# jinhan/tacotron2-vae

Measured on AMD Instinct MI355X. Metric: mel-frames/s (train step, batch=6, 80-mel), higher is better.
Workload: dtype f32; 1 GPU; configs[1]: Tacotron2-VAE fp32 train step (fwd+loss+bwd+clip+Adam), B=6/GPU fixed shape T_in=84 T_out=400, dropout on, random-init seed 1234; step_mode=hip-graph replay, decoder_forward=persistent, decoder_backward=persistent, startup_steps=43, global_batch=6, parallelism=dp1

## Files before the change

### tacotron2-vae_amd/csrc/conv_gemm.hip

```cpp
#include <stdlib.h>
#include <type_traits>
#include "t2v_common.h"
#include "t2v_kernels.h"
#include "t2v_coop.h"
#include "t2v_x3.h"


#define CG_BM 64
#define CG_BN 64
#define CG_BK 32

struct ConvGemmArgs {
    const float* W;
    const float* X;
    const float* dY;
    const float* bias;
    float* Y;
    float* stat_part;
    int B, Cin, T, M, KS;
};

template <int MODE, int KS>
__global__ __launch_bounds__(256) void k_conv_gemm(ConvGemmArgs a) {
    __shared__ float As[2][CG_BK][CG_BM + 1];
// ... 157 lines not shown
        if (second_ == 0u) return;
        if (tid == 0) __hip_atomic_store(a.ks_ctr + tile, 0u, __ATOMIC_RELAXED, __HIP_MEMORY_SCOPE_AGENT);
        const float* other = a.ks_part + (((1 - blockIdx.z) * ntile + tile) * 256 + tid) * (4 * NTW);
        float o[NTW][4];
#pragma unroll
        for (int n = 0; n < NTW; ++n)
#pragma unroll
            for (int r = 0; r < 4; ++r) o[n][r] = ld_sc1(other + 4 * n + r);
#pragma unroll
        for (int n = 0; n < NTW; ++n)
#pragma unroll
            for (int r = 0; r < 4; ++r) acc[n][r] += o[n][r];
    }
    float psum[4] = {0.f, 0.f, 0.f, 0.f}, psq[4] = {0.f, 0.f, 0.f, 0.f};
#pragma unroll
    for (int r = 0; r < 4; ++r) {
        const int m = m0 + 16 * wave + 4 * kq + r;
        if (m < a.M) {
            const float bv = a.bias ? a.bias[m] : 0.f;
            float* yrow = a.Y + ((size_t)bb * a.M + m) * a.T;
#pragma unroll
            for (int n = 0; n < NTW; ++n) {
                const int t = t0 + 16 * n + j;
                if (t < a.T) {
                    const float v = acc[n][r] + bv;
                    yrow[t] = v;
                    psum[r] += v;
                    psq[r] = fmaf(v, v, psq[r]);
                }
            }
        }
    }
    if (a.stat_part) {
#pragma unroll
        for (int r = 0; r < 4; ++r) {
            const float s1 = row16_sum(psum[r]), s2 = row16_sum(psq[r]);
            const int m = m0 + 16 * wave + 4 * kq + r;
            if (j == 0 && m < a.M) {
                float* dst = a.stat_part + ((size_t)blockIdx.x * a.M + m) * 2;
                dst[0] = s1;
                dst[1] = s2;
            }
        }
    }
}

template <int NTW>
__global__ __launch_bounds__(256) void k_conv5_fwd(ConvTiledArgs a) {
    constexpr int BN = 16 * NTW;
    constexpr int XW = BN + 4;
    constexpr int XS = BN == 32 ? 48 : BN <= 64 ? 80 : 112;
    constexpr int NX = (16 * XW + 255) / 256;
    __shared__ float As[2][CT_KT][CT_AS];
    __shared__ float Xs[2][16][XS];
    const int tid = threadIdx.x, wave = tid >> 6, lane = tid & 63;
    const int kq = lane >> 4, j = lane & 15;
    const int bb = blockIdx.x / a.tiles_per_item, t0 = (blockIdx.x % a.tiles_per_item) * BN;
    const int m0 = blockIdx.y * CT_BM;
    const int CK = a.Cin * 5;
    const int nkt_all = a.Cin / 16;
    const int kt0 = gridDim.z > 1 ? (int)blockIdx.z * (nkt_all / 2) : 0;
    const int nkt = gridDim.z > 1 ? (blockIdx.z == 0 ? nkt_all / 2 : nkt_all - nkt_all / 2) : nkt_all;

    const bool stamp = a.prof && tid == 0 && blockIdx.x == 0 && blockIdx.y == 0 && blockIdx.z == 0;
    if (stamp) { a.prof[0] = __builtin_readcyclecounter(); a.prof[2] = wall_clock64(); }
    float4 ra[5];
    float rx[NX];
    const int a_m = tid & 63, w4 = tid >> 6;
    const float* a_row = a.W + (size_t)min(m0 + a_m, a.M - 1) * CK + 4 * w4;
    int a_lds[20];
#pragma unroll
    for (int q = 0; q < 20; ++q) {
        const int k = 4 * w4 + 16 * (q >> 2) + (q & 3);
        const int c = k / 5, kx = k - 5 * c;
        a_lds[q] = (16 * kx + c) * CT_AS + a_m;
    }
    const float* x_item = a.X + (size_t)bb * a.Cin * a.T;
    int x_goff[NX], x_lds[NX];
    bool x_ok[NX];
#pragma unroll
    for (int i = 0; i < NX; ++i) {
        const int e = tid + 256 * i;
        const int c = min(e / XW, 15), jj = e - (e / XW) * XW;
        const int t = t0 - 2 + jj;
        x_ok[i] = e < 16 * XW && t >= 0 && t < a.T;
        x_goff[i] = c * a.T + min(max(t, 0), a.T - 1);
        x_lds[i] = e < 16 * XW ? c * XS + jj : -1;
    }
    auto load_one = [&](int kt, int q) {
        if (q < 5) {
            ra[q] = *(const float4*)(a_row + 80 * (kt0 + kt) + 16 * q);
        } else {
            const float v = x_item[(size_t)16 * (kt0 + kt) * a.T + x_goff[q - 5]];
            rx[q - 5] = x_ok[q - 5] ? v : 0.f;
        }
    };
    auto store_one = [&](int buf, int q) {
        if (q < 20) {
            const float4 v4 = ra[q >> 2];
            const float v = (q & 3) == 0 ? v4.x : (q & 3) == 1 ? v4.y : (q & 3) == 2 ? v4.z : v4.w;
            (&As[buf][0][0])[a_lds[q]] = v;
        } else if (q < 20 + NX) {
            if (x_lds[q - 20] >= 0) (&Xs[buf][0][0])[x_lds[q - 20]] = rx[q - 20];
        }
    };
    constexpr int NLOAD = 5 + NX, NSTORE = 20 + NX;
    constexpr int S_ST0 = 11;
    static_assert(NLOAD <= S_ST0 + 1 && NSTORE <= 3 * (20 - S_ST0), "side work must fit the k-steps");

    f32x4 acc[NTW];
#pragma unroll
    for (int n = 0; n < NTW; ++n) acc[n] = f32x4{0.f, 0.f, 0.f, 0.f};
#pragma unroll
    for (int q = 0; q < NLOAD; ++q) load_one(0, q);
#pragma unroll
    for (int q = 0; q < NSTORE; ++q) store_one(0, q);
    __syncthreads();
    for (int kt = 0; kt < nkt; ++kt) {
        const int buf = kt & 1;
        const int kn = min(kt + 1, nkt - 1);
        const float* ap = &As[buf][kq][16 * wave + j];
        const float* xp = &Xs[buf][kq][j];
        float av[2], bv[2][NTW];
        av[0] = ap[0];
#pragma unroll
        for (int n = 0; n < NTW; ++n) bv[0][n] = xp[16 * n];
#pragma unroll
        for (int s = 0; s < 20; ++s) {
            if (s < NLOAD) load_one(kn, s);
            if (s + 1 < 20) {
                av[(s + 1) & 1] = ap[4 * (s + 1) * CT_AS];
#pragma unroll
                for (int n = 0; n < NTW; ++n)
                    bv[(s + 1) & 1][n] = xp[4 * ((s + 1) & 3) * XS + 16 * n + ((s + 1) >> 2)];
            }
            __builtin_amdgcn_sched_barrier(0);
#pragma unroll
            for (int n = 0; n < NTW; ++n) acc[n] = mfma16x4(av[s & 1], bv[s & 1][n], acc[n]);
            __builtin_amdgcn_sched_barrier(0);
            if (s >= S_ST0) {
#pragma unroll
                for (int q = 3 * (s - S_ST0); q < 3 * (s - S_ST0) + 3; ++q) store_one(buf ^ 1, q);
                __builtin_amdgcn_sched_barrier(0);
            }
        }
        __syncthreads();
    }
    if (stamp) { a.prof[1] = __builtin_readcyclecounter(); a.prof[3] = wall_clock64(); }
    conv5_fwd_finish<NTW>(a, acc, bb, t0, m0);
}

#define CD_RING 3
#define CD_AS 84
__device__ float g_conv5_zero[4];

template <int NTW>
__global__ __launch_bounds__(256) void k_conv5_fwd_dma(ConvTiledArgs a) {
    constexpr int BN = 16 * NTW;
    constexpr int XW = BN + 4;
    constexpr int XS = BN == 32 ? 48 : BN <= 64 ? 80 : 112;
    constexpr int NXD = 16 * XS / 256;
    constexpr int G = 6 + NXD;
    constexpr int AST = CT_BM * CD_AS, STG = AST + 16 * XS;
    static_assert(16 * XS % 256 == 0 && AST % 256 == 0, "whole 64-lane requests");
    __shared__ __attribute__((aligned(16))) float lds_[CD_RING * STG];
    const unsigned lds0 = (unsigned)(unsigned long)(__attribute__((address_space(3))) void*)&lds_[0];
    const int tid = threadIdx.x, wave = __builtin_amdgcn_readfirstlane(tid >> 6), lane = tid & 63;
    const int kq = lane >> 4, j = lane & 15;
    const int bb = blockIdx.x / a.tiles_per_item, t0 = (blockIdx.x % a.tiles_per_item) * BN;
    const int m0 = blockIdx.y * CT_BM;
    const int CK = a.Cin * 5;
    const int nkt_all = a.Cin / 16;
    const int kt0 = gridDim.z > 1 ? (int)blockIdx.z * (nkt_all / 2) : 0;
    const int nkt = gridDim.z > 1 ? (blockIdx.z == 0 ? nkt_all / 2 : nkt_all - nkt_all / 2) : nkt_all;

    const bool stamp = a.prof && tid == 0 && blockIdx.x == 0 && blockIdx.y == 0 && blockIdx.z == 0;
    if (stamp) { a.prof[0] = __builtin_readcyclecounter(); a.prof[2] = wall_clock64(); }
    const float* a_ptr[6];
#pragma unroll
    for (int i = 0; i < 6; ++i) {
        const int u = 64 * min(wave + 4 * i, 20) + lane;
        const int row = u / 21, pc = u - 21 * row;
        a_ptr[i] = a.W + (size_t)min(m0 + row, a.M - 1) * CK + 80 * kt0 + 4 * min(pc, 19);
    }
    const float* x_ptr[NXD];
    size_t x_step[NXD];
#pragma unroll
    for (int i = 0; i < NXD; ++i) {
        const int e = 64 * (wave + 4 * i) + lane;
        const int c = e / XS, jj = e - c * XS;
        const int t = t0 - 2 + jj;
        const bool ok = jj < XW && t >= 0 && t < a.T;
        x_ptr[i] = ok ? a.X + ((size_t)bb * a.Cin + 16 * kt0 + c) * a.T + t : g_conv5_zero;
        x_step[i] = ok ? (size_t)16 * a.T : 0;
    }
    auto request = [&](unsigned dst, int q) {
        if (q < 5) {
            t2v_dma16(a_ptr[q], dst + 1024u * (unsigned)wave + 4096u * q);
            a_ptr[q] += 80;
        } else if (q == 5) {
            t2v_dma16(a_ptr[5], dst + 20480u);
            a_ptr[5] += 80;
        } else if (q < G) {
            t2v_dma4(x_ptr[q - 6], dst + 4u * AST + 256u * (unsigned)wave + 1024u * (q - 6));
            x_ptr[q - 6] += x_step[q - 6];
        }
    };

    f32x4 acc[NTW];
#pragma unroll
    for (int n = 0; n < NTW; ++n) acc[n] = f32x4{0.f, 0.f, 0.f, 0.f};
#pragma unroll
    for (int q = 0; q < G; ++q) request(lds0, q);
    if (nkt > 1) {
#pragma unroll
        for (int q = 0; q < G; ++q) request(lds0 + 4u * STG, q);
    }
    if (nkt > 1) t2v_wait_vmcnt<G>(); else t2v_wait_vmcnt<0>();
    __syncthreads();
    constexpr int CD_SYNC = 10;
    constexpr int TWO = G > 20 - CD_SYNC ? G - (20 - CD_SYNC) : 0;
    static_assert(G <= 2 * (20 - CD_SYNC) && (TWO == 0 || NTW >= 3), "a tile's requests fit the steps behind the barrier");
    const int lane_a = CD_AS * (16 * wave + j) + 5 * kq, lane_x = AST + kq * XS + j;
    float av[2], bv[2][NTW];
    auto fetch = [&](const float* ap, const float* xp, int s) {
        av[s & 1] = ap[20 * (s & 3) + (s >> 2)];
#pragma unroll
        for (int n = 0; n < NTW; ++n) bv[s & 1][n] = xp[4 * (s & 3) * XS + 16 * n + (s >> 2)];
    };
    auto tile = [&](auto more_c, const float* ap, const float* xp, const float* ap1, const float* xp1, unsigned dst2) {
        constexpr bool MORE = decltype(more_c)::value;
#pragma unroll
        for (int s = 0; s < 20; ++s) {
            if (s == CD_SYNC) {
                t2v_wait_vmcnt<0>();
                __syncthreads();
                __builtin_amdgcn_sched_barrier(0);
            }
            const int sr = s - CD_SYNC;
            const int q0 = !MORE || sr < 0 ? -1 : sr < TWO ? 2 * sr : sr + TWO;
            const int q1 = MORE && sr >= 0 && sr < TWO ? 2 * sr + 1 : -1;
#pragma unroll
            for (int n = 0; n < NTW; ++n) {
                acc[n] = mfma16x4(av[s & 1], bv[s & 1][n], acc[n]);
                __builtin_amdgcn_sched_barrier(0);
                if (n == 0) { if (s + 1 < 20) fetch(ap, xp, s + 1); else fetch(ap1, xp1, 0); }
                if (n == 1 && q0 >= 0 && q0 < G) request(dst2, q0);
                if (n == 2 && q1 >= 0) request(dst2, q1);
                __builtin_amdgcn_sched_barrier(0);
            }
        }
    };
    fetch(&lds_[lane_a], &lds_[lane_x], 0);
    int stg = 0;
    for (int kt = 0; kt < nkt; ++kt) {
        const int stg1 = stg == CD_RING - 1 ? 0 : stg + 1, stg2 = stg == 0 ? CD_RING - 1 : stg - 1;
        const float* ap = &lds_[stg * STG + lane_a];
        const float* xp = &lds_[stg * STG + lane_x];
        const float* ap1 = &lds_[stg1 * STG + lane_a];
        const float* xp1 = &lds_[stg1 * STG + lane_x];
        if (kt + 2 < nkt) tile(std::true_type{}, ap, xp, ap1, xp1, lds0 + 4u * (unsigned)(stg2 * STG));
        else tile(std::false_type{}, ap, xp, ap1, xp1, 0u);
        stg = stg1;
    }
    if (stamp) { a.prof[1] = __builtin_readcyclecounter(); a.prof[3] = wall_clock64(); }
    conv5_fwd_finish<NTW>(a, acc, bb, t0, m0);
}

template <int BT>
__global__ __launch_bounds__(256) void k_conv5_dw(ConvTiledArgs a) {
    constexpr int XW = BT + 4;
    constexpr int XS = (BT == 80) ? 100 : 116;
    constexpr int NA = BT / 16;
    constexpr int NX = (16 * XW + 255) / 256;
    __shared__ float As[2][BT][CT_AS];
    __shared__ float Xs[2][16][XS];
    const int tid = threadIdx.x, wave = tid >> 6, lane = tid & 63;
    const int kq = lane >> 4, j = lane & 15;
    const int c0 = blockIdx.x * 16, m0 = blockIdx.y * CT_BM;
    const int CK = a.Cin * 5;
    const int tiles = (a.T + BT - 1) / BT, nkt_all = a.B * tiles;
    const int per = (nkt_all + gridDim.z - 1) / gridDim.z;
    const int kt_lo = blockIdx.z * per, kt_hi = min(nkt_all, kt_lo + per);
    const bool vec = (a.T & 3) == 0;

    float4 ra[NA];
    float rx[NX];
    const int a_m = tid & 63;
    const bool a_ok = m0 + a_m < a.M;
    auto load_tiles = [&](int kt) {
        const int bb = kt / tiles, t0 = (kt - bb * tiles) * BT;
        const float* arow = a.dY + ((size_t)bb * a.M + (a_ok ? m0 + a_m : 0)) * a.T;
#pragma unroll
        for (int i = 0; i < NA; ++i) {
            const int t = t0 + 4 * ((tid >> 6) + 4 * i);
            float4 v = make_float4(0.f, 0.f, 0.f, 0.f);
            if (a_ok) {
                if (vec) {
                    if (t < a.T) v = *(const float4*)(arow + t);
                } else {
                    if (t < a.T) v.x = arow[t];
                    if (t + 1 < a.T) v.y = arow[t + 1];
                    if (t + 2 < a.T) v.z = arow[t + 2];
                    if (t + 3 < a.T) v.w = arow[t + 3];
                }
            }
            ra[i] = v;
        }
        const float* x_item = a.X + ((size_t)bb * a.Cin + c0) * a.T;
#pragma unroll
        for (int i = 0; i < NX; ++i) {
            const int e = tid + 256 * i;
            const int c = e / XW, jj = e - c * XW;
            const int t = t0 - 2 + jj;
            rx[i] = (c < 16 && t >= 0 && t < a.T) ? x_item[(size_t)c * a.T + t] : 0.f;
        }
    };
    auto store_tiles = [&](int buf) {
#pragma unroll
        for (int i = 0; i < NA; ++i) {
            const int k = 4 * ((tid >> 6) + 4 * i);
            As[buf][k][a_m] = ra[i].x;
            As[buf][k + 1][a_m] = ra[i].y;
            As[buf][k + 2][a_m] = ra[i].z;
            As[buf][k + 3][a_m] = ra[i].w;
        }
#pragma unroll
        for (int i = 0; i < NX; ++i) {
            const int e = tid + 256 * i;
            const int c = e / XW, jj = e - c * XW;
            if (c < 16) Xs[buf][c][jj] = rx[i];
        }
    };

    int boff[5];
#pragma unroll
    for (int n = 0; n < 5; ++n) {
        const int nl = 16 * n + j, c = nl / 5, kx = nl - 5 * c;
        boff[n] = c * XS + kx + kq;
    }
    f32x4 acc[5];
#pragma unroll
    for (int n = 0; n < 5; ++n) acc[n] = f32x4{0.f, 0.f, 0.f, 0.f};
    if (kt_lo < kt_hi) {
        load_tiles(kt_lo);
        store_tiles(0);
    }
    __syncthreads();
    for (int kt = kt_lo; kt < kt_hi; ++kt) {
        const int buf = (kt - kt_lo) & 1;
        if (kt + 1 < kt_hi) load_tiles(kt + 1);
        const float* ap = &As[buf][kq][16 * wave + j];
        const float* xp = &Xs[buf][0][0];
        float av[2], bv[2][5];
        av[0] = ap[0];
#pragma unroll
        for (int n = 0; n < 5; ++n) bv[0][n] = xp[boff[n]];
#pragma unroll
        for (int s = 0; s < BT / 4; ++s) {
            if (s + 1 < BT / 4) {
                av[(s + 1) & 1] = ap[4 * (s + 1) * CT_AS];
#pragma unroll
                for (int n = 0; n < 5; ++n) bv[(s + 1) & 1][n] = xp[boff[n] + 4 * (s + 1)];
            }
            __builtin_amdgcn_sched_barrier(0);
#pragma unroll
            for (int n = 0; n < 5; ++n) acc[n] = mfma16x4(av[s & 1], bv[s & 1][n], acc[n]);
            __builtin_amdgcn_sched_barrier(0);
        }
        if (kt + 1 < kt_hi) store_tiles(buf ^ 1);
        __syncthreads();
    }
#pragma unroll
    for (int r = 0; r < 4; ++r) {
        const int m = m0 + 16 * wave + 4 * kq + r;
        if (m < a.M) {
            float* drow = a.Y + (size_t)blockIdx.z * a.M * CK + (size_t)m * CK + 5 * c0;
#pragma unroll
            for (int n = 0; n < 5; ++n) drow[16 * n + j] = acc[n][r];
        }
    }
}

#define CB_RS 24

__global__ void k_conv5_pack_bf16(const float* __restrict__ W, unsigned short* __restrict__ Wp, int M, int Cin, int flipT) {
    const int R = flipT ? Cin : M, Cc = flipT ? M : Cin;
    const size_t i = (size_t)blockIdx.x * blockDim.x + threadIdx.x;
    if (i >= (size_t)R * Cc * 5) return;
    const int c16 = i & 15, kx = (i >> 4) % 5;
    const size_t rc = (i >> 4) / 5;
    const int cb = rc % (Cc / 16), r = rc / (Cc / 16);
    const int cc = 16 * cb + c16;
    const float v = flipT ? W[((size_t)cc * Cin + r) * 5 + (4 - kx)] : W[((size_t)r * Cin + cc) * 5 + kx];
    const __bf16 b = (__bf16)v;
    Wp[i] = *(const unsigned short*)&b;
}

struct ConvBf16Args {
    const unsigned short* Wp;
    const float* X;
    const float* bias;
    float* Y;
    float* stat_part;
    int B, Cin, T, M, tiles_per_item;
};

template <int NTW>
__global__ __launch_bounds__(256) void k_conv5_fwd_bf16(ConvBf16Args a) {
    constexpr int BN = 16 * NTW;
    constexpr int XW = BN + 4;
    constexpr int NXP = (8 * XW + 255) / 256;
    __shared__ __attribute__((aligned(16))) unsigned short As[2][5][CT_BM][CB_RS];
    __shared__ __attribute__((aligned(16))) unsigned short Xt[2][XW][CB_RS];
    const int tid = threadIdx.x, wave = tid >> 6, lane = tid & 63;
    const int kq = lane >> 4, j = lane & 15;
    const int bb = blockIdx.x / a.tiles_per_item, t0 = (blockIdx.x % a.tiles_per_item) * BN;
    const int m0 = blockIdx.y * CT_BM;
    const int ncb = a.Cin / 16;

    uint4 ra[3];
    const unsigned short* a_src[3];
    int a_lds[3];
#pragma unroll
    for (int i = 0; i < 3; ++i) {
        const int q = tid + 256 * i;
        const int row = min(q / 10, CT_BM - 1), ch = q - (q / 10) * 10;
        a_src[i] = a.Wp + (size_t)min(m0 + row, a.M - 1) * ncb * 80 + ch * 8;
        a_lds[i] = q < 640 ? (((ch >> 1) * CT_BM + row) * CB_RS + 8 * (ch & 1)) : -1;
    }
    float rx[NXP][2];
    const float* x_item = a.X + (size_t)bb * a.Cin * a.T;
    int x_goff[NXP], x_lds[NXP];
    bool x_ok[NXP];
#pragma unroll
    for (int i = 0; i < NXP; ++i) {
        const int e = tid + 256 * i;
        const int cp = min(e / XW, 7), pos = e - (e / XW) * XW;
        const int t = t0 - 2 + pos;
        x_ok[i] = e < 8 * XW && t >= 0 && t < a.T;
        x_goff[i] = 2 * cp * a.T + min(max(t, 0), a.T - 1);
        x_lds[i] = e < 8 * XW ? pos * CB_RS + 2 * cp : -1;
    }
    auto load_tiles = [&](int kt) {
#pragma unroll
        for (int i = 0; i < 3; ++i) ra[i] = *(const uint4*)(a_src[i] + 80 * kt);
#pragma unroll
        for (int i = 0; i < NXP; ++i) {
            const float* px = x_item + (size_t)16 * kt * a.T + x_goff[i];
            const float v0 = px[0], v1 = px[a.T];
            rx[i][0] = x_ok[i] ? v0 : 0.f;
            rx[i][1] = x_ok[i] ? v1 : 0.f;
        }
    };
    auto store_tiles = [&](int buf) {
#pragma unroll
        for (int i = 0; i < 3; ++i)
            if (a_lds[i] >= 0) *(uint4*)(&As[buf][0][0][0] + a_lds[i]) = ra[i];
#pragma unroll
        for (int i = 0; i < NXP; ++i)
            if (x_lds[i] >= 0) *(unsigned*)(&Xt[buf][0][0] + x_lds[i]) = t2v_pack_bf16x2(rx[i][0], rx[i][1]);
    };

    f32x4 acc[NTW];
#pragma unroll
    for (int n = 0; n < NTW; ++n) acc[n] = f32x4{0.f, 0.f, 0.f, 0.f};
    load_tiles(0);
    store_tiles(0);
    __syncthreads();
    for (int kt = 0; kt < ncb; ++kt) {
        const int buf = kt & 1;
        load_tiles(min(kt + 1, ncb - 1));
#pragma unroll
        for (int kx = 0; kx < 5; ++kx) {
            const t2v_s16x4 av = *(const t2v_s16x4*)&As[buf][kx][16 * wave + j][4 * kq];
#pragma unroll
            for (int n = 0; n < NTW; ++n) {
                const t2v_s16x4 bv = *(const t2v_s16x4*)&Xt[buf][16 * n + j + kx][4 * kq];
                acc[n] = __builtin_amdgcn_mfma_f32_16x16x16bf16_1k(av, bv, acc[n], 0, 0, 0);
            }
        }
        store_tiles(buf ^ 1);
        __syncthreads();
    }

    float psum[4] = {0.f, 0.f, 0.f, 0.f}, psq[4] = {0.f, 0.f, 0.f, 0.f};
#pragma unroll
    for (int r = 0; r < 4; ++r) {
        const int m = m0 + 16 * wave + 4 * kq + r;
        if (m < a.M) {
            const float bv = a.bias ? a.bias[m] : 0.f;
            float* yrow = a.Y + ((size_t)bb * a.M + m) * a.T;
#pragma unroll
            for (int n = 0; n < NTW; ++n) {
                const int t = t0 + 16 * n + j;
                if (t < a.T) {
                    const float v = acc[n][r] + bv;
                    yrow[t] = v;
                    psum[r] += v;
                    psq[r] = fmaf(v, v, psq[r]);
                }
            }
        }
    }
    if (a.stat_part) {
#pragma unroll
        for (int r = 0; r < 4; ++r) {
            const float s1 = row16_sum(psum[r]), s2 = row16_sum(psq[r]);
            const int m = m0 + 16 * wave + 4 * kq + r;
            if (j == 0 && m < a.M) {
                float* dst = a.stat_part + ((size_t)blockIdx.x * a.M + m) * 2;
                dst[0] = s1;
                dst[1] = s2;
            }
        }
    }
}

#define CB2_RS 40
template <int NTW>
__global__ __launch_bounds__(256) void k_conv5_fwd_bf16k32(ConvBf16Args a) {
    constexpr int BN = 16 * NTW;
    constexpr int XW = BN + 4;
    constexpr int NXP = (16 * XW + 255) / 256;
    __shared__ __attribute__((aligned(16))) unsigned short As[2][5][CT_BM][CB2_RS];
// ... 333 lines not shown
        if (BN == 32) k_conv5_fwd_dma<2><<<grid, 256, 0, stream>>>(a);
        else if (BN == 48) k_conv5_fwd_dma<3><<<grid, 256, 0, stream>>>(a);
        else if (BN == 64) k_conv5_fwd_dma<4><<<grid, 256, 0, stream>>>(a);
        else if (BN == 80) k_conv5_fwd_dma<5><<<grid, 256, 0, stream>>>(a);
        else k_conv5_fwd_dma<6><<<grid, 256, 0, stream>>>(a);
        return;
    }
    if (BN == 32) k_conv5_fwd<2><<<grid, 256, 0, stream>>>(a);
    else if (BN == 48) k_conv5_fwd<3><<<grid, 256, 0, stream>>>(a);
    else if (BN == 64) k_conv5_fwd<4><<<grid, 256, 0, stream>>>(a);
    else if (BN == 80) k_conv5_fwd<5><<<grid, 256, 0, stream>>>(a);
    else k_conv5_fwd<6><<<grid, 256, 0, stream>>>(a);
}

static void launch_conv5_fwd_bf16(const float* W, int flipT, unsigned short* Wp, const float* X, const float* bias,
                                  float* Y, float* stat_part, int B, int Cin, int T, int M, int W_M, int W_Cin,
                                  hipStream_t stream) {
    const size_t n = (size_t)W_M * W_Cin * 5;
    k_conv5_pack_bf16<<<(unsigned)((n + 255) / 256), 256, 0, stream>>>(W, Wp, W_M, W_Cin, flipT);
    int ks_unused = 1;
    const int BN = conv5_pick_bn_ks(T, B, M, Cin, &ks_unused);
    ConvBf16Args a;
    a.Wp = Wp; a.X = X; a.bias = bias; a.Y = Y; a.stat_part = stat_part;
    a.B = B; a.Cin = Cin; a.T = T; a.M = M; a.tiles_per_item = (T + BN - 1) / BN;
    dim3 grid(B * a.tiles_per_item, (M + CT_BM - 1) / CT_BM);
    static const int k32 = getenv("T2V_CONV_BF16_K32") ? atoi(getenv("T2V_CONV_BF16_K32")) : 1;
    if (k32 && Cin % 32 == 0) {
        if (BN == 32) k_conv5_fwd_bf16k32<2><<<grid, 256, 0, stream>>>(a);
        else if (BN == 48) k_conv5_fwd_bf16k32<3><<<grid, 256, 0, stream>>>(a);
        else if (BN == 64) k_conv5_fwd_bf16k32<4><<<grid, 256, 0, stream>>>(a);
        else if (BN == 80) k_conv5_fwd_bf16k32<5><<<grid, 256, 0, stream>>>(a);
        else k_conv5_fwd_bf16k32<6><<<grid, 256, 0, stream>>>(a);
        return;
    }
    if (BN == 32) k_conv5_fwd_bf16<2><<<grid, 256, 0, stream>>>(a);
    else if (BN == 48) k_conv5_fwd_bf16<3><<<grid, 256, 0, stream>>>(a);
    else if (BN == 64) k_conv5_fwd_bf16<4><<<grid, 256, 0, stream>>>(a);
    else if (BN == 80) k_conv5_fwd_bf16<5><<<grid, 256, 0, stream>>>(a);
    else k_conv5_fwd_bf16<6><<<grid, 256, 0, stream>>>(a);
}

__global__ void k_conv_flip_weight(const float* __restrict__ W, float* __restrict__ Wt, int M, int Cin, int KS) {
    const int i = blockIdx.x * blockDim.x + threadIdx.x;
    if (i >= M * Cin * KS) return;
    const int k = i % KS, c = (i / KS) % Cin, m = i / (KS * Cin);
    Wt[((size_t)c * M + m) * KS + (KS - 1 - k)] = W[i];
}

struct ConvFlipBatch { const float* W[16]; float* Wt[16]; int M[16]; int Cin[16]; int n; int KS; };
__global__ void k_conv_flip_weight_batched(ConvFlipBatch f) {
    const int l = blockIdx.y;
    const int M = f.M[l], Cin = f.Cin[l], KS = f.KS;
    const float* __restrict__ W = f.W[l];
    float* __restrict__ Wt = f.Wt[l];
    const int n = M * Cin * KS;
    for (int i = blockIdx.x * blockDim.x + threadIdx.x; i < n; i += gridDim.x * blockDim.x) {
        const int k = i % KS, c = (i / KS) % Cin, m = i / (KS * Cin);
        Wt[((size_t)c * M + m) * KS + (KS - 1 - k)] = W[i];
    }
}

extern "C" int t2v_conv1d_flip_weights(const float* const* W, float* const* Wt, const int* Cout, const int* Cin, int KS,
                                       int n, void* stream_) {
    hipStream_t stream = (hipStream_t)stream_;
    if (!W || !Wt || !Cout || !Cin || n < 1 || n > 16 || KS < 1) return T2V_ERR_ARG;
    ConvFlipBatch f;
    f.n = n; f.KS = KS;
    int mx = 0;
    for (int i = 0; i < n; ++i) {
        if (!W[i] || !Wt[i] || Cout[i] < 1 || Cin[i] < 1) return T2V_ERR_ARG;
        f.W[i] = W[i]; f.Wt[i] = Wt[i]; f.M[i] = Cout[i]; f.Cin[i] = Cin[i];
        mx = max(mx, Cout[i] * Cin[i] * KS);
    }
    const int bx = min(1024, (mx + 1023) / 1024);
    k_conv_flip_weight_batched<<<dim3(bx, n), 256, 0, stream>>>(f);
    return t2v_check_launch();
}

extern "C" int t2v_conv1d_fwd(const float* W, const float* X, const float* bias, float* Y, float* stat_part,
                              int B, int Cin, int T, int Cout, int KS, void* stream_) {
    hipStream_t stream = (hipStream_t)stream_;
    if (!W || !X || !Y || B < 1 || Cin < 1 || T < 1 || Cout < 1 || KS < 1 || !(KS & 1)) return T2V_ERR_ARG;
    if (t2v_conv5_x3_ok(B, Cin, T, Cout, KS)) {
        const int rc = t2v_conv5_x3_run(W, X, bias, Y, stat_part, B, Cin, T, Cout, stream, 3);
        return rc != T2V_OK ? rc : t2v_check_launch();
    }
    if (conv5_tiled_ok(Cin, KS)) {
        launch_conv5_fwd(W, X, bias, Y, stat_part, B, Cin, T, Cout, stream);
        return t2v_check_launch();
    }
    ConvGemmArgs a;
    a.W = W; a.X = X; a.dY = nullptr; a.bias = bias; a.Y = Y; a.stat_part = stat_part;
    a.B = B; a.Cin = Cin; a.T = T; a.M = Cout; a.KS = KS;
    dim3 grid((B * T + CG_BN - 1) / CG_BN, (Cout + CG_BM - 1) / CG_BM);
    if (KS == 5) k_conv_gemm<0, 5><<<grid, 256, 0, stream>>>(a);
    else if (KS == 3) k_conv_gemm<0, 3><<<grid, 256, 0, stream>>>(a);
    else return T2V_ERR_DIMS;
    return t2v_check_launch();
}

extern "C" int t2v_conv1d_stat_blocks(int B, int T, int Cin, int Cout, int KS) {
    if (t2v_conv5_x3_ok(B, Cin, T, Cout, KS)) return t2v_conv5_x3_stat_blocks(B, T);
    if (conv5_tiled_ok(Cin, KS)) { int ks; const int BN = conv5_pick_bn_ks(T, B, Cout, Cin, &ks); return B * ((T + BN - 1) / BN); }
    return (B * T + CG_BN - 1) / CG_BN;
}

extern "C" int t2v_conv1d_stat_blocks_bf16(int B, int T, int Cin, int Cout, int KS) {
    if (t2v_conv5_planes_bf16_ok(B, Cin, T, Cout, KS)) return t2v_conv5_x3_stat_blocks(B, T);
    if (conv5_tiled_ok(Cin, KS)) { int ks; const int BN = conv5_pick_bn_ks(T, B, Cout, Cin, &ks); return B * ((T + BN - 1) / BN); }
    return (B * T + CG_BN - 1) / CG_BN;
}

extern "C" int t2v_conv1d_dw_scratch_floats(int B, int Cin, int T, int Cout, int KS) {
    if (!conv5_tiled_ok(Cin, KS)) return 0;
    const int ns = conv5_dw_splits(B, Cin, T, Cout, true);
    return ns > 1 ? ns * Cout * Cin * 5 : 0;
}

static thread_local bool g_conv_dw_bf16 = false;
extern "C" int t2v_conv1d_bwd(const float* W, const float* X, const float* dY, float* dX, float* dW, float* Wt_scratch,
                              float* dw_scratch, int B, int Cin, int T, int Cout, int KS, void* stream_) {
    hipStream_t stream = (hipStream_t)stream_;
    if (!X || !dY || B < 1 || Cin < 1 || T < 1 || Cout < 1 || KS < 1 || !(KS & 1)) return T2V_ERR_ARG;
    if (dX) {
        if (!Wt_scratch) return T2V_ERR_ARG;
        const int n = Cout * Cin * KS;
        if (W) k_conv_flip_weight<<<(n + 255) / 256, 256, 0, stream>>>(W, Wt_scratch, Cout, Cin, KS);
        if (t2v_conv5_x3_ok(B, Cout, T, Cin, KS)) {
            const int rc = t2v_conv5_x3_run(Wt_scratch, dY, nullptr, dX, nullptr, B, Cout, T, Cin, stream, 3);
            if (rc != T2V_OK) return rc;
        } else if (conv5_tiled_ok(Cout, KS)) {
            launch_conv5_fwd(Wt_scratch, dY, nullptr, dX, nullptr, B, Cout, T, Cin, stream);
        } else {
            ConvGemmArgs a;
            a.W = Wt_scratch; a.X = dY; a.dY = nullptr; a.bias = nullptr; a.Y = dX; a.stat_part = nullptr;
            a.B = B; a.Cin = Cout; a.T = T; a.M = Cin; a.KS = KS;
            dim3 grid((B * T + CG_BN - 1) / CG_BN, (Cin + CG_BM - 1) / CG_BM);
            if (KS == 5) k_conv_gemm<0, 5><<<grid, 256, 0, stream>>>(a);
            else if (KS == 3) k_conv_gemm<0, 3><<<grid, 256, 0, stream>>>(a);
            else return T2V_ERR_DIMS;
        }
    }
    if (dW && conv5_tiled_ok(Cin, KS)) {
        const bool dw_bf16 = g_conv_dw_bf16;
        ConvTiledArgs a;
        a.W = nullptr; a.X = X; a.dY = dY; a.bias = nullptr; a.Y = dW; a.stat_part = nullptr;
        a.B = B; a.Cin = Cin; a.T = T; a.M = Cout; a.tiles_per_item = 0;
        a.prof = nullptr; a.ks_part = nullptr; a.ks_ctr = nullptr;
        const int ns = conv5_dw_splits(B, Cin, T, Cout, dw_bf16);
        if (ns > 1 && !dw_scratch) return T2V_ERR_ARG;
        if (ns > 1) a.Y = dw_scratch;
        dim3 grid(Cin / 16, (Cout + CT_BM - 1) / CT_BM, ns);
        const int c80 = ((T + 79) / 80) * 80, c96 = ((T + 95) / 96) * 96;
        if (dw_bf16) {
            if (c80 <= c96) k_conv5_dw_bf16<80><<<grid, 256, 0, stream>>>(a);
            else k_conv5_dw_bf16<96><<<grid, 256, 0, stream>>>(a);
        } else if (c80 <= c96) k_conv5_dw<80><<<grid, 256, 0, stream>>>(a);
        else k_conv5_dw<96><<<grid, 256, 0, stream>>>(a);
        if (ns > 1) {
            const int n = Cout * Cin * 5;
            k_conv5_dw_reduce<<<(n + 255) / 256, 256, 0, stream>>>(dw_scratch, dW, n, ns);
        }
    } else if (dW) {
        ConvGemmArgs a;
        a.W = nullptr; a.X = X; a.dY = dY; a.bias = nullptr; a.Y = dW; a.stat_part = nullptr;
        a.B = B; a.Cin = Cin; a.T = T; a.M = Cout; a.KS = KS;
        dim3 grid((Cin * KS + CG_BN - 1) / CG_BN, (Cout + CG_BM - 1) / CG_BM);
        if (KS == 5) k_conv_gemm<1, 5><<<grid, 256, 0, stream>>>(a);
        else if (KS == 3) k_conv_gemm<1, 3><<<grid, 256, 0, stream>>>(a);
        else return T2V_ERR_DIMS;
    }
    return t2v_check_launch();
}

extern "C" int t2v_conv1d_fwd_bf16(const float* W, const float* X, const float* bias, float* Y, float* stat_part,
                                   void* Wp_scratch, int B, int Cin, int T, int Cout, int KS, void* stream_) {
    hipStream_t stream = (hipStream_t)stream_;
    if (!W || !X || !Y || !Wp_scratch || B < 1 || Cin < 1 || T < 1 || Cout < 1) return T2V_ERR_ARG;
    if (!conv5_tiled_ok(Cin, KS)) return T2V_ERR_DIMS;
    if (t2v_conv5_planes_bf16_ok(B, Cin, T, Cout, KS)) {
        const int rc = t2v_conv5_x3_run(W, X, bias, Y, stat_part, B, Cin, T, Cout, stream, 1);
        return rc != T2V_OK ? rc : t2v_check_launch();
    }
    launch_conv5_fwd_bf16(W, 0, (unsigned short*)Wp_scratch, X, bias, Y, stat_part, B, Cin, T, Cout, Cout, Cin, stream);
    return t2v_check_launch();
}

extern "C" int t2v_conv1d_bwd_bf16(const float* W, const float* X, const float* dY, float* dX, float* dW,
                                   void* Wp_scratch, float* dw_scratch, int B, int Cin, int T, int Cout, int KS,
                                   void* stream_) {
    hipStream_t stream = (hipStream_t)stream_;
    if (!X || !dY || B < 1 || Cin < 1 || T < 1 || Cout < 1) return T2V_ERR_ARG;
    if (!conv5_tiled_ok(Cin, KS) || (dX && !conv5_tiled_ok(Cout, KS))) return T2V_ERR_DIMS;
    if (dX) {
        if (!W || !Wp_scratch) return T2V_ERR_ARG;
        bool done = false;
        if (t2v_conv5_planes_bf16_ok(B, Cout, T, Cin, KS)) {
            float* wt = conv_ks_scratch((size_t)Cout * Cin * KS);
            if (wt) {
                k_conv_flip_weight<<<(Cout * Cin * KS + 255) / 256, 256, 0, stream>>>(W, wt, Cout, Cin, KS);
                const int rc = t2v_conv5_x3_run(wt, dY, nullptr, dX, nullptr, B, Cout, T, Cin, stream, 1);
                if (rc != T2V_OK) return rc;
                done = true;
            }
        }
        if (!done) launch_conv5_fwd_bf16(W, 1, (unsigned short*)Wp_scratch, dY, nullptr, dX, nullptr, B, Cout, T, Cin, Cout, Cin, stream);
    }
    if (dW) {
        g_conv_dw_bf16 = true;
        const int rc = t2v_conv1d_bwd(W, X, dY, nullptr, dW, nullptr, dw_scratch, B, Cin, T, Cout, KS, stream_);
        g_conv_dw_bf16 = false;
        return rc;
    }
    return t2v_check_launch();
}
```

### tacotron2-vae_amd/csrc/t2v_x3.h

```cpp
#pragma once
#include "t2v_common.h"

__device__ __forceinline__ void t2v_split8(const float (&v)[8], uint4& p0, uint4& p1, uint4& p2) {
    unsigned q0[4], q1[4], q2[4];
#pragma unroll
    for (int c = 0; c < 4; ++c) {
        const float x = v[2 * c], y = v[2 * c + 1];
        const unsigned h = t2v_pack_bf16x2(x, y);
        const float r1x = x - __uint_as_float(h << 16), r1y = y - __uint_as_float(h & 0xffff0000u);
        const unsigned m = t2v_pack_bf16x2(r1x, r1y);
        const float r2x = r1x - __uint_as_float(m << 16), r2y = r1y - __uint_as_float(m & 0xffff0000u);
        q0[c] = h; q1[c] = m; q2[c] = t2v_pack_bf16x2(r2x, r2y);
    }
    p0 = make_uint4(q0[0], q0[1], q0[2], q0[3]);
    p1 = make_uint4(q1[0], q1[1], q1[2], q1[3]);
    p2 = make_uint4(q2[0], q2[1], q2[2], q2[3]);
}

__device__ __forceinline__ void t2v_dma16(const void* gsrc, unsigned lds_addr) {
    unsigned keep;
    asm volatile("s_mov_b32 %0, m0\n\ts_mov_b32 m0, %2\n\ts_nop 0\n\tglobal_load_lds_dwordx4 %1, off\n\ts_mov_b32 m0, %0"
                 : "=&s"(keep) : "v"(gsrc), "s"(lds_addr) : "memory");
}

__device__ __forceinline__ void t2v_dma4(const void* gsrc, unsigned lds_addr) {
    unsigned keep;
    asm volatile("s_mov_b32 %0, m0\n\ts_mov_b32 m0, %2\n\ts_nop 0\n\tglobal_load_lds_dword %1, off\n\ts_mov_b32 m0, %0"
                 : "=&s"(keep) : "v"(gsrc), "s"(lds_addr) : "memory");
}

template <int N>
__device__ __forceinline__ void t2v_wait_vmcnt() {
    if constexpr (N == 0) asm volatile("s_waitcnt vmcnt(0)" ::: "memory");
    else if constexpr (N == 4) asm volatile("s_waitcnt vmcnt(4)" ::: "memory");
    else if constexpr (N == 6) asm volatile("s_waitcnt vmcnt(6)" ::: "memory");
    else if constexpr (N == 7) asm volatile("s_waitcnt vmcnt(7)" ::: "memory");
    else if constexpr (N == 8) asm volatile("s_waitcnt vmcnt(8)" ::: "memory");
    else if constexpr (N == 9) asm volatile("s_waitcnt vmcnt(9)" ::: "memory");
    else if constexpr (N == 10) asm volatile("s_waitcnt vmcnt(10)" ::: "memory");
    else if constexpr (N == 11) asm volatile("s_waitcnt vmcnt(11)" ::: "memory");
    else if constexpr (N == 12) asm volatile("s_waitcnt vmcnt(12)" ::: "memory");
    else if constexpr (N == 13) asm volatile("s_waitcnt vmcnt(13)" ::: "memory");
    else if constexpr (N == 14) asm volatile("s_waitcnt vmcnt(14)" ::: "memory");
    else if constexpr (N == 16) asm volatile("s_waitcnt vmcnt(16)" ::: "memory");
    else static_assert(N == 0, "add the literal");
}
```

Baseline: 231,000 mel-frames/s.

## Add DMA-staged multi-stage ring pipeline for conv5 weight-gradient kernel

Adds a new conv5 weight-gradient kernel that streams dY and X tiles straight into LDS with global_load_lds in a 5-stage ring. Loads are issued in half-tiles interleaved between MFMA steps, with vmcnt waits and one barrier per stage. The goal is to hide global memory latency and cut the register round-trip staging of the old kernel. It runs by default for fp32 dW when T is divisible by 4 and the pointers are 16-byte aligned, at the cost of complex hand scheduling and added LDS use.

```diff
diff --git a/tacotron2-vae_amd/csrc/conv_gemm.hip b/tacotron2-vae_amd/csrc/conv_gemm.hip
--- a/tacotron2-vae_amd/csrc/conv_gemm.hip
+++ b/tacotron2-vae_amd/csrc/conv_gemm.hip
@@ -333,7 +333,7 @@
 
 #define CD_RING 3
 #define CD_AS 84
-__device__ float g_conv5_zero[4];
+__device__ __attribute__((aligned(16))) float g_conv5_zero[4];
 
 template <int NTW>
 __global__ __launch_bounds__(256) void k_conv5_fwd_dma(ConvTiledArgs a) {
@@ -552,6 +552,180 @@
         if (kt + 1 < kt_hi) store_tiles(buf ^ 1);
         __syncthreads();
     }
+#pragma unroll
+    for (int r = 0; r < 4; ++r) {
+        const int m = m0 + 16 * wave + 4 * kq + r;
+        if (m < a.M) {
+            float* drow = a.Y + (size_t)blockIdx.z * a.M * CK + (size_t)m * CK + 5 * c0;
+#pragma unroll
+            for (int n = 0; n < 5; ++n) drow[16 * n + j] = acc[n][r];
+        }
+    }
+}
+
+#define CW_RING 5
+template <int BT>
+__global__ __launch_bounds__(256) void k_conv5_dw_dma(ConvTiledArgs a) {
+    constexpr int HT = BT / 2, NS = HT / 4;
+    constexpr int AP = HT / 4 + 1, AS = 4 * AP;
+    constexpr int XW = HT + 4, XS = BT == 80 ? 48 : 52;
+    constexpr int NAR = AP, NXR = 16 * XS / 64;
+    constexpr int NAD = (NAR + 3) / 4, NXD = (NXR + 3) / 4, G = NAD + NXD;
+    constexpr int AST = CT_BM * AS, STG = AST + 16 * XS;
+    static_assert(16 * XS % 64 == 0 && XS >= XW && STG % 4 == 0 && AST % 4 == 0, "whole requests, aligned stages");
+    __shared__ __attribute__((aligned(16))) float lds_[CW_RING * STG];
+    const unsigned lds0 = (unsigned)(unsigned long)(__attribute__((address_space(3))) void*)&lds_[0];
+    const int tid = threadIdx.x, wave = __builtin_amdgcn_readfirstlane(tid >> 6), lane = tid & 63;
+    const int kq = lane >> 4, j = lane & 15;
+    const int c0 = blockIdx.x * 16, m0 = blockIdx.y * CT_BM;
+    const int CK = a.Cin * 5;
+    const int tiles = (a.T + BT - 1) / BT, nkt_all = a.B * tiles;
+    const int per = (nkt_all + gridDim.z - 1) / gridDim.z;
+    const int kt_lo = blockIdx.z * per, kt_hi = min(nkt_all, kt_lo + per);
+    const int nu = 2 * max(kt_hi - kt_lo, 0);
+
+    const bool stamp = a.prof && tid == 0 && blockIdx.x == 0 && blockIdx.y == 0 && blockIdx.z == 0;
+    if (stamp) { a.prof[0] = __builtin_readcyclecounter(); a.prof[2] = wall_clock64(); }
+    const float* a_src[NAD];
+    int a_lim[NAD];
+    unsigned a_dst[NAD];
+#pragma unroll
+    for (int i = 0; i < NAD; ++i) {
+        const int r = min(wave + 4 * i, NAR - 1);
+        const int u = 64 * r + lane, row = u / AP, pc = min(u - AP * row, AP - 2);
+        a_src[i] = a.dY + (size_t)min(m0 + row, a.M - 1) * a.T + 4 * pc;
+        a_lim[i] = a.T - 4 * pc;
+        a_dst[i] = 1024u * (unsigned)r;
+    }
+    const float* x_src[NXD];
+    int x_j[NXD];
+    unsigned x_dst[NXD];
+#pragma unroll
+    for (int i = 0; i < NXD; ++i) {
+        const int r = min(wave + 4 * i, NXR - 1);
+        const int e = 64 * r + lane, c = e / XS, jj = e - c * XS;
+        x_src[i] = a.X + ((ptrdiff_t)(c0 + c) * a.T + (jj - 2));
+        x_j[i] = jj < XW ? jj - 2 : 0x40000000;
+        x_dst[i] = 4u * AST + 256u * (unsigned)r;
+    }
+    const int t_end = 2 * tiles * HT;
+    int rq_t;
+    ptrdiff_t rq_a, rq_x;
+    {
+        const int bb = kt_lo / tiles;
+        rq_t = (kt_lo - bb * tiles) * BT;
+        rq_a = (ptrdiff_t)bb * a.M * a.T + rq_t;
+        rq_x = (ptrdiff_t)bb * a.Cin * a.T + rq_t;
+    }
+    const ptrdiff_t a_wrap = (ptrdiff_t)a.M * a.T - t_end, x_wrap = (ptrdiff_t)a.Cin * a.T - t_end;
+    auto advance = [&]() {
+        rq_t += HT; rq_a += HT; rq_x += HT;
+        if (rq_t == t_end) { rq_t = 0; rq_a += a_wrap; rq_x += x_wrap; }
+    };
+    auto source = [&](int q) -> const float* {
+        if (q < NAD) return rq_t < a_lim[q] ? a_src[q] + rq_a : g_conv5_zero;
+        return (unsigned)(rq_t + x_j[q - NAD]) < (unsigned)a.T ? x_src[q - NAD] + rq_x : g_conv5_zero;
+    };
+    auto issue = [&](unsigned dst, int q, const float* src) {
+        if (q < NAD) t2v_dma16(src, __builtin_amdgcn_readfirstlane(dst + a_dst[q]));
+        else t2v_dma4(src, __builtin_amdgcn_readfirstlane(dst + x_dst[q - NAD]));
+    };
+
+    int boff[5];
+#pragma unroll
+    for (int n = 0; n < 5; ++n) {
+        const int nl = 16 * n + j, c = nl / 5, kx = nl - 5 * c;
+        boff[n] = AST + c * XS + kx + kq;
+    }
+    const int lane_a = AS * (16 * wave + j) + kq;
+    f32x4 acc[5];
+#pragma unroll
+    for (int n = 0; n < 5; ++n) acc[n] = f32x4{0.f, 0.f, 0.f, 0.f};
+    typedef const __attribute__((address_space(3))) float* lds_p;
+    auto lds_at = [&](unsigned byte_addr) -> lds_p { asm volatile("" : "+v"(byte_addr)); return (lds_p)(size_t)byte_addr; };
+    static_assert(NS % 2 == 0, "k-steps are fetched in pairs");
+    float av[NS], bv[NS][5];
+    constexpr int CW_SYNC = NS / 2;
+    constexpr int TWO = G - (NS - CW_SYNC);
+    static_assert(TWO >= 0 && TWO <= NS - CW_SYNC, "a stage's requests fit the steps behind the barrier");
+    auto stage = [&](auto v_c, unsigned sb, unsigned sb1, unsigned dst4) {
+        constexpr int V = decltype(v_c)::value;
+        constexpr bool MORE = V == 3;
+        const lds_p pa = lds_at(sb + 4u * lane_a), pa1 = lds_at(sb1 + 4u * lane_a);
+        lds_p pb[5], pb1[5];
+#pragma unroll
+        for (int n = 0; n < 5; ++n) { pb[n] = lds_at(sb + 4u * boff[n]); pb1[n] = lds_at(sb1 + 4u * boff[n]); }
+        auto pair = [&](int s2, int half) {
+            const bool nx = s2 >= NS;
+            const int t = nx ? s2 - NS : s2;
+            if (half == 0) {
+                const lds_p q = nx ? pa1 : pa;
+                av[t] = q[4 * t]; av[t + 1] = q[4 * t + 4];
+            }
+#pragma unroll
+            for (int n = half ? 2 : 0; n < (half ? 5 : 2); ++n) {
+                const lds_p q = nx ? pb1[n] : pb[n];
+                bv[t][n] = q[4 * t]; bv[t + 1][n] = q[4 * t + 4];
+            }
+        };
+        const float* src = nullptr;
+#pragma unroll
+        for (int s = 0; s < NS; ++s) {
+            if (s == CW_SYNC) {
+                if constexpr (V >= 2) t2v_wait_vmcnt<2 * G>();
+                else if constexpr (V == 1) t2v_wait_vmcnt<G>();
+                else t2v_wait_vmcnt<0>();
+                __syncthreads();
+                __builtin_amdgcn_sched_barrier(0);
+            }
+            const int sr = s - CW_SYNC;
+            const int q0 = !MORE || sr < 0 ? -1 : sr < TWO ? 2 * sr : sr + TWO;
+            const int q1 = MORE && sr >= 0 && sr < TWO ? 2 * sr + 1 : -1;
+#pragma unroll
+            for (int n = 0; n < 5; ++n) {
+                acc[n] = mfma16x4(av[s], bv[s][n], acc[n]);
+                __builtin_amdgcn_sched_barrier(0);
+                if (n == 0) pair((s & ~1) + 2, s & 1);
+                if (n == 1 && q0 >= 0) src = source(q0);
+                if (n == 2 && q0 >= 0) issue(dst4, q0, src);
+                if (n == 3 && q1 >= 0) src = source(q1);
+                if (n == 4 && q1 >= 0) issue(dst4, q1, src);
+                __builtin_amdgcn_sched_barrier(0);
+            }
+        }
+        if constexpr (MORE) advance();
+    };
+    if (nu > 0) {
+        const int np = min(nu, CW_RING - 1);
+        for (int p = 0; p < np; ++p) {
+#pragma unroll
+            for (int q = 0; q < G; ++q) issue(lds0 + 4u * (unsigned)(p * STG), q, source(q));
+            advance();
+        }
+        if (np >= 4) t2v_wait_vmcnt<3 * G>();
+        else if (np == 3) t2v_wait_vmcnt<2 * G>();
+        else if (np == 2) t2v_wait_vmcnt<G>();
+        else t2v_wait_vmcnt<0>();
+        __syncthreads();
+#pragma unroll
+        for (int s = 0; s < 2; ++s) {
+            av[s] = lds_[lane_a + 4 * s];
+#pragma unroll
+            for (int n = 0; n < 5; ++n) bv[s][n] = lds_[boff[n] + 4 * s];
+        }
+        int stg = 0;
+        for (int u = 0; u < nu; ++u) {
+            const int stg1 = stg == CW_RING - 1 ? 0 : stg + 1, stg4 = stg == 0 ? CW_RING - 1 : stg - 1;
+            const unsigned sb = lds0 + 4u * (unsigned)(stg * STG), sb1 = lds0 + 4u * (unsigned)(stg1 * STG);
+            const int left = nu - 2 - u;
+            if (left > 2) stage(std::integral_constant<int, 3>{}, sb, sb1, lds0 + 4u * (unsigned)(stg4 * STG));
+            else if (left == 2) stage(std::integral_constant<int, 2>{}, sb, sb1, 0u);
+            else if (left == 1) stage(std::integral_constant<int, 1>{}, sb, sb1, 0u);
+            else stage(std::integral_constant<int, 0>{}, sb, sb1, 0u);
+            stg = stg1;
+        }
+    }
+    if (stamp) { a.prof[1] = __builtin_readcyclecounter(); a.prof[3] = wall_clock64(); }
 #pragma unroll
     for (int r = 0; r < 4; ++r) {
         const int m = m0 + 16 * wave + 4 * kq + r;
@@ -1191,9 +1365,16 @@
         if (ns > 1) a.Y = dw_scratch;
         dim3 grid(Cin / 16, (Cout + CT_BM - 1) / CT_BM, ns);
         const int c80 = ((T + 79) / 80) * 80, c96 = ((T + 95) / 96) * 96;
+        static const int staging = getenv("T2V_CONV_STAGING") ? atoi(getenv("T2V_CONV_STAGING")) : 1;
+        static const int dw_staging = getenv("T2V_CONV_DW_STAGING") ? atoi(getenv("T2V_CONV_DW_STAGING")) : 1;
+        const bool dw_dma = !dw_bf16 && staging && dw_staging && T % 4 == 0 && (((uintptr_t)dY | (uintptr_t)X) & 15) == 0;
         if (dw_bf16) {
             if (c80 <= c96) k_conv5_dw_bf16<80><<<grid, 256, 0, stream>>>(a);
             else k_conv5_dw_bf16<96><<<grid, 256, 0, stream>>>(a);
+        } else if (dw_dma) {
+            a.prof = g_t2v_prof;
+            if (c80 <= c96) k_conv5_dw_dma<80><<<grid, 256, 0, stream>>>(a);
+            else k_conv5_dw_dma<96><<<grid, 256, 0, stream>>>(a);
         } else if (c80 <= c96) k_conv5_dw<80><<<grid, 256, 0, stream>>>(a);
         else k_conv5_dw<96><<<grid, 256, 0, stream>>>(a);
         if (ns > 1) {
diff --git a/tacotron2-vae_amd/csrc/t2v_x3.h b/tacotron2-vae_amd/csrc/t2v_x3.h
--- a/tacotron2-vae_amd/csrc/t2v_x3.h
+++ b/tacotron2-vae_amd/csrc/t2v_x3.h
@@ -43,5 +43,7 @@
     else if constexpr (N == 13) asm volatile("s_waitcnt vmcnt(13)" ::: "memory");
     else if constexpr (N == 14) asm volatile("s_waitcnt vmcnt(14)" ::: "memory");
     else if constexpr (N == 16) asm volatile("s_waitcnt vmcnt(16)" ::: "memory");
+    else if constexpr (N == 18) asm volatile("s_waitcnt vmcnt(18)" ::: "memory");
+    else if constexpr (N == 24) asm volatile("s_waitcnt vmcnt(24)" ::: "memory");
     else static_assert(N == 0, "add the literal");
 }
```

Result: no change. 232,000 mel-frames/s, median of 6 (+0.4%).
